# kkbwilldo/quantizations

Hardware: AMD Instinct MI355X
Metric: decode tokens/sec Llama-3-8B NF4 bs=1; 4096×4096 GEMV GB/s vs HBM peak (higher is better)
Workload: dtype f16 activations x 4-bit NF4 weights (exact NF4 codes (fp32 as hi+lo fp16)), fp32 accumulate; 1 GPU; llama3-8b-nf4-dq-decode-bs1; layers=32, prompt_len=32, global_batch=1, stream_batch=1, decode=hipgraph, parallelism=single, projection_groups=64, layer_ops=229, compute_dtype=fp32, rmsnorm_in_grouped_gemv=True, decode_attention=qz_decode_attention, silu_in_gate_up_launch=True, residual_in_gemv_epilogue=True, lm_head=layer_ops.gemv_dense, lm_head_rows_split=False, attention=single GPU

## Files before the change

### quantizations_amd/csrc/diag_stamps.hip

```cpp
#define QZ_STAMPS 1
#include "gemv.hip"

#define QZ_DIAG_API extern "C" __attribute__((visibility("default")))

QZ_DIAG_API int qz_diag_set_stamp_buffer(unsigned long long *buf) {
  return (int)hipMemcpyToSymbol(HIP_SYMBOL(g_qz_stamp), &buf, sizeof(buf));
}

QZ_DIAG_API int qz_diag_gemv_stamped(int M, int K, const void *x, const unsigned char *B, int exact,
                                     const unsigned char *qabsmax, const float *absmax2, const float *code2,
                                     const float *offset, void *y, int *nwaves, void *stream) {
  GemvParams p;
  bool vec_ok;
  const int st = make_params(M, K, x, QZ_DT_F16, B, QZ_NF4, 64, nullptr, qabsmax, absmax2, code2, offset, 256, 0,
                             nullptr, nullptr, y, &p, &vec_ok);
  if (st != QZ_OK) return st;
  if (!vec_ok || !full_steps(K, 64, 256, true, 0) || !nwaves) return QZ_ERR_SHAPE;
  int R, WK;
  choose_geometry(M, K, QZ_DT_F16, &R, &WK);
  if (WK != 1 || (R != 2 && R != 4)) return QZ_ERR_SHAPE;
  set_tables(QZ_NF4, nullptr, exact != 0, QZ_DT_F16, &p);
  const unsigned grid = (unsigned)((M + R * 4 - 1) / (R * 4));
  hipStream_t s = (hipStream_t)stream;
  const bool two = two_steps(K, 1, true);
#define QZ_DG(RR, CL_, TWO_) \
  hipLaunchKernelGGL((k_gemv_4bit<true, QZ_DT_F16, RR, 1, 4, true, CL_, false, TWO_, 2>), dim3(grid), dim3(256), 0, s, p)
#define QZ_DG2(RR, CL_) do { if (two) QZ_DG(RR, CL_, true); else QZ_DG(RR, CL_, false); } while (0)
  if (R == 2) { if (exact) QZ_DG2(2, true); else QZ_DG2(2, false); }
  else { if (exact) QZ_DG2(4, true); else QZ_DG2(4, false); }
#undef QZ_DG2
#undef QZ_DG
  QZ_LAUNCH_CHECK();
  *nwaves = (int)grid * 4;
  return QZ_OK;
}
```

### quantizations_amd/csrc/gemv.hip

```cpp
#include "gemv_launch.h"

namespace qz {

static int env_int(const char *name, int dflt) {
  const char *e = getenv(name);
  return e && *e ? atoi(e) : dflt;
}
static Knobs read_knobs() {
  Knobs k;
  k.wide8 = env_int("QZ_GEMV_WIDE8", 1) != 0;
  const int nr = env_int("QZ_GROUPED_NORM_R", 0);
  k.norm_r = (nr == 1 || nr == 2 || nr == 4) ? nr : 0;
  const int pr = env_int("QZ_PAIR_R", 0);
  k.pair_r = (pr == 2 || pr == 3 || pr == 4 || pr == 6 || pr == 8) ? pr : 0;
  k.pair_wt = env_int("QZ_PAIR_WT", 1) != 0;
  k.pair_ps = env_int("QZ_PAIR_PS", -1);
  k.pair_wk1 = env_int("QZ_PAIR_WK1", 2);
  return k;
}
static Knobs g_knobs = read_knobs();
Knobs &gemv_knobs() { return g_knobs; }
static int g_gemm16_sched = env_int("QZ_GEMM16_SCHED", 971);
int &gemm16_sched() { return g_gemm16_sched; }


template <bool DQ, int DT, int R, bool CL, bool NRM, bool TWO, bool PS = false, bool WT = false>
__global__ __launch_bounds__(256) void k_gemv_4bit_pair(GemvGroup g) {
  const int wave = __builtin_amdgcn_readfirstlane((int)threadIdx.x / kWave);
  const GemvParams seg = g.seg[wave >> 1];
  gemv_body<DQ, DT, R, 1, 4, true, CL, WT, NRM, true, TWO, PS>(seg, blockIdx.x, g.seg);
}

}

using namespace qz;

extern "C" int qz_gemv_4bit(int M, int K, const void *x, int dtype, const unsigned char *B, int quant_type,
                            int blocksize, const float *absmax, const unsigned char *qabsmax, const float *absmax2,
                            const float *code2, const float *offset, int blocksize2, long long block_base,
                            const float *lut, const void *bias, void *y, void *stream) {
  return gemv_impl<false>(M, K, x, dtype, B, quant_type, blocksize, absmax, qabsmax, absmax2, code2, offset,
                          blocksize2, block_base, lut, bias, nullptr, nullptr, y, stream);
}

extern "C" int qz_gemv_4bit_residual(int M, int K, const void *x, int dtype, const unsigned char *B, int quant_type,
                                     int blocksize, const float *absmax, const unsigned char *qabsmax,
                                     const float *absmax2, const float *code2, const float *offset, int blocksize2,
                                     long long block_base, const float *lut, const void *bias, const void *residual,
                                     void *y, void *stream) {
  if (!residual) return QZ_ERR_ARG;
  return gemv_impl<false>(M, K, x, dtype, B, quant_type, blocksize, absmax, qabsmax, absmax2, code2, offset,
                          blocksize2, block_base, lut, bias, residual, nullptr, y, stream);
}

extern "C" int qz_gemv_4bit_grouped(int nseg, const qz_gemv_segment *segs, int K, const void *x, int dtype,
                                    int quant_type, int blocksize, int blocksize2, const float *lut, void *stream) {
  return gemv_grouped_impl<false>(nseg, segs, nullptr, nullptr, K, x, dtype, quant_type, blocksize, blocksize2, lut,
                                  nullptr, 0.0f, stream);
}

extern "C" int qz_gemv_4bit_grouped_rmsnorm(int nseg, const qz_gemv_segment *segs, int K, const void *x, int dtype,
                                            int quant_type, int blocksize, int blocksize2, const float *lut,
                                            const void *norm_weight, float eps, void *stream) {
  if (!norm_weight || !x) return QZ_ERR_ARG;
  return gemv_grouped_impl<false>(nseg, segs, nullptr, nullptr, K, x, dtype, quant_type, blocksize, blocksize2, lut,
                                  norm_weight, eps, stream);
}

template <bool DQ, int DT, int R, bool CL, bool NRM>
static void launch_pair_wt(unsigned grid, size_t lds, hipStream_t s, const GemvGroup &g, bool two) {
  if constexpr (CL && NRM && DT == QZ_DT_F16 && (R == 2 || R == 4)) {
    if (two) hipLaunchKernelGGL((k_gemv_4bit_pair<DQ, DT, R, CL, NRM, true, true, true>), dim3(grid), dim3(256), lds, s, g);
    else hipLaunchKernelGGL((k_gemv_4bit_pair<DQ, DT, R, CL, NRM, false, true, true>), dim3(grid), dim3(256), lds, s, g);
  }
}

template <bool DQ, int DT, int R, bool CL, bool NRM>
static void launch_pair_ps_loop(unsigned grid, int blocks, size_t lds, hipStream_t s, const GemvGroup &g) {
  if constexpr (NRM)
    hipLaunchKernelGGL((k_gemv_4bit_pair<DQ, DT, R, CL, NRM, false, true>), dim3(grid), dim3(256), lds, s, g);
  else
    hipLaunchKernelGGL((k_gemv_4bit_pair<DQ, DT, R, CL, NRM, false>), dim3(blocks), dim3(256), lds, s, g);
}

extern "C" int qz_gemv_4bit_pair_silu(const qz_gemv_segment *segs, int K, const void *x, int dtype, int quant_type,
                                      int blocksize, int blocksize2, const float *lut, const void *norm_weight,
                                      float eps, void *h, void *stream) {
  if (!segs || !h || !x) return QZ_ERR_ARG;
  if (segs[0].M != segs[1].M) return QZ_ERR_SHAPE;
  if (dtype != QZ_DT_F16 && dtype != QZ_DT_BF16) return QZ_ERR_SHAPE;
  GemvGroup g;
  g.nseg = 2;
  const bool cl = exact_codes(quant_type, lut) && dtype == QZ_DT_F16;
  const bool dq = segs[0].qabsmax != nullptr;
  for (int i = 0; i < 2; ++i) {
// ... 1 lines not shown
    bool v;
    const int st = make_params(q.M, K, x, dtype, q.B, quant_type, blocksize, q.absmax, q.qabsmax, q.absmax2, q.code2,
                               q.offset, blocksize2, q.block_base, lut, q.bias, h, &g.seg[i], &v);
    if (st != QZ_OK) return st;
    if ((q.qabsmax != nullptr) != dq || !v || !full_steps(K, blocksize, blocksize2, dq, q.block_base))
      return QZ_ERR_SHAPE;
    set_tables(quant_type & ~QZ_EXACT_CODES, lut, cl, dtype, &g.seg[i]);
    g.seg[i].nw = norm_weight;
    g.seg[i].eps = eps;
  }
  const int M = segs[0].M;
  if (M == 0) return QZ_OK;
  if (norm_weight && (K % 8 != 0 || K > 16384 || ((uintptr_t)x | (uintptr_t)norm_weight) % 16 != 0))
    return QZ_ERR_SHAPE;
  int R, WK;
  choose_geometry(2 * M, K, dtype, &R, &WK);
  if (WK != 1) {
    const int wk1 = gemv_knobs().pair_wk1;
    if (wk1 == 0 || (norm_weight && wk1 != 2)) return QZ_ERR_SHAPE;
    WK = 1;
  }
  if (gemv_knobs().pair_r) R = gemv_knobs().pair_r;
  const int blocks = (M + 2 * R - 1) / (2 * R);
  if (norm_weight && blocks > kNormMaxBlocks) return QZ_ERR_SHAPE;
  for (int i = 2; i < kMaxSeg; ++i) g.start[i] = 0;
  hipStream_t s = (hipStream_t)stream;
  const size_t lds = norm_weight ? (size_t)K * 2 : 0;
  const bool two = two_steps(K, 1, true);
  const int cus = device_cus();
  const size_t img = norm_weight ? (size_t)K * 2 : 0;
  const int per_cu_wt = (int)std::min<size_t>(3, kLdsPerCU / (2 * kTabDwords * 4 + img + 4096));
  const int per_cu = (int)std::min<size_t>(3, kLdsPerCU / (kTabDwords * 4 + img + 4096));
  const bool wt_ok = cl && norm_weight && (R == 2 || R == 4) && blocks >= 3 * 2 * cus && per_cu_wt >= 2 &&
                     gemv_knobs().pair_wt;
  int pgrid_i = 0;
  if (gemv_knobs().pair_ps >= 0) {
    const int ps = gemv_knobs().pair_ps;
    pgrid_i = ps <= 0 ? 0 : ps <= 8 ? cus * ps : ps;
  } else if (norm_weight) {
    pgrid_i = (wt_ok ? 2 : per_cu) * cus;
  }
  const unsigned pgrid = (unsigned)max(pgrid_i, 1);
  const bool persist = pgrid_i > 0 && pgrid_i < blocks;
  const bool pair_wt = persist && wt_ok;
#define QZ_PS(DQ_, DT_, RR, CL_, NRM_)                                                                               \
  do {                                                                                                              \
    if (pair_wt) launch_pair_wt<DQ_, DT_, RR, CL_, NRM_>(pgrid, lds, s, g, two);                                        \
    else if (persist && two) hipLaunchKernelGGL((k_gemv_4bit_pair<DQ_, DT_, RR, CL_, NRM_, true, true>), dim3(pgrid), \
                                                dim3(256), lds, s, g);                                              \
    else if (persist) launch_pair_ps_loop<DQ_, DT_, RR, CL_, NRM_>(pgrid, blocks, lds, s, g);                      \
    else if (two) hipLaunchKernelGGL((k_gemv_4bit_pair<DQ_, DT_, RR, CL_, NRM_, true>), dim3(blocks), dim3(256),    \
                                     lds, s, g);                                                                    \
    else hipLaunchKernelGGL((k_gemv_4bit_pair<DQ_, DT_, RR, CL_, NRM_, false>), dim3(blocks), dim3(256), lds, s, g); \
  } while (0)
#define QZ_PS_R(DQ_, DT_, CL_, NRM_)                  \
  do {                                                \
    if (R == 4) QZ_PS(DQ_, DT_, 4, CL_, NRM_);        \
    else if (R == 8) QZ_PS(DQ_, DT_, 8, CL_, NRM_);   \
    else if (R == 6) QZ_PS(DQ_, DT_, 6, CL_, NRM_);   \
    else if (R == 3) QZ_PS(DQ_, DT_, 3, CL_, NRM_);   \
    else if (R == 1) QZ_PS(DQ_, DT_, 1, CL_, NRM_);   \
    else QZ_PS(DQ_, DT_, 2, CL_, NRM_);               \
  } while (0)
#define QZ_PS_N(DQ_, DT_, CL_)                                                         \
  do {                                                                                 \
    if (norm_weight) QZ_PS_R(DQ_, DT_, CL_, true); else QZ_PS_R(DQ_, DT_, CL_, false); \
  } while (0)
  if (dtype == QZ_DT_F16) {
    if (dq) { if (cl) QZ_PS_N(true, QZ_DT_F16, true); else QZ_PS_N(true, QZ_DT_F16, false); }
    else { if (cl) QZ_PS_N(false, QZ_DT_F16, true); else QZ_PS_N(false, QZ_DT_F16, false); }
  } else {
    if (dq) QZ_PS_N(true, QZ_DT_BF16, false); else QZ_PS_N(false, QZ_DT_BF16, false);
  }
#undef QZ_PS_N
#undef QZ_PS_R
#undef QZ_PS
  QZ_LAUNCH_CHECK();
  return QZ_OK;
}

extern "C" int qz_gemv_knobs(char *buf, int n) {
  char tmp[320];
  const int len = snprintf(tmp, sizeof(tmp),
                           "{\"QZ_GEMV_WIDE8\": %d, \"QZ_GROUPED_NORM_R\": %d, \"QZ_PAIR_R\": %d, \"QZ_PAIR_WT\": %d, "
                           "\"QZ_PAIR_PS\": %d, \"QZ_PAIR_WK1\": %d, \"QZ_GEMM16_SCHED\": %d, \"cus\": %d}",
                           gemv_knobs().wide8, gemv_knobs().norm_r, gemv_knobs().pair_r, gemv_knobs().pair_wt,
                           gemv_knobs().pair_ps, gemv_knobs().pair_wk1, gemm16_sched(), device_cus());
  if (buf && n > len) memcpy(buf, tmp, (size_t)len + 1);
  return len;
}

extern "C" int qz_gemv_set_knob(const char *name, int value) {
  if (!name) return QZ_ERR_ARG;
  Knobs &k = gemv_knobs();
  if (!strcmp(name, "QZ_GEMV_WIDE8")) k.wide8 = value != 0;
  else if (!strcmp(name, "QZ_GROUPED_NORM_R")) k.norm_r = (value == 1 || value == 2 || value == 4) ? value : 0;
  else if (!strcmp(name, "QZ_PAIR_R")) k.pair_r = (value == 2 || value == 3 || value == 4 || value == 6 || value == 8) ? value : 0;
  else if (!strcmp(name, "QZ_PAIR_WT")) k.pair_wt = value != 0;
  else if (!strcmp(name, "QZ_PAIR_PS")) k.pair_ps = value;
  else if (!strcmp(name, "QZ_PAIR_WK1")) k.pair_wk1 = value;
  else if (!strcmp(name, "QZ_GEMM16_SCHED")) gemm16_sched() = value;
  else return QZ_ERR_ARG;
  return QZ_OK;
}
```

### quantizations_amd/csrc/gemv_core.h

```cpp
#pragma once
#include "common.h"

#include <atomic>
#include <cstdio>
#include <cstdlib>
#include <cstring>

namespace qz {

constexpr int kTabCopies = 32;
constexpr int kTabDwords = 256 * kTabCopies;
constexpr int kTabCopiesCL = 16;

constexpr uint16_t f16_bits_rne_c(float f) {
  const uint32_t u = __builtin_bit_cast(uint32_t, f);
  const uint32_t sign = (u >> 16) & 0x8000u, au = u & 0x7FFFFFFFu;
  if (au == 0) return (uint16_t)sign;
  const uint32_t e = (au >> 23) - 127u + 15u, m = au & 0x7FFFFFu;
  uint32_t h = (e << 10) | (m >> 13);
  const uint32_t rem = m & 0x1FFFu;
  if (rem > 0x1000u || (rem == 0x1000u && (h & 1u))) h += 1u;
  return (uint16_t)(sign | h);
}
struct ByteTable {
// ... 324 lines not shown
    store_byte_table_entry<PIECES>(s_tab, u32x4{h, l, h, l}, (uint32_t)e);
  }
}

template <int NT, int PIECES = kTabCopies / 4>
__device__ __forceinline__ void build_byte_table_f32(uint32_t *s_tab, const float *lut) {
  for (int e = threadIdx.x; e < 256; e += NT) {
    const uint32_t a = __float_as_uint(lut[e >> 4]), b = __float_as_uint(lut[e & 15]);
    store_byte_table_entry<PIECES>(s_tab, u32x4{a, b, a, b}, (uint32_t)e);
  }
}

template <bool DQ, int DT, int R, bool NOX, bool FS> struct StepLoads {
  static constexpr int kXWords = DT == QZ_DT_F32 ? 32 : 16;
  u32x4 wv[R];
  uint32_t q[R];
  float a[R];
  uint32_t xr[kXWords];
  int xb;
  bool on;

  __device__ __forceinline__ void load_x(const void *x, uint32_t e0) {
    const u32x4 *p = reinterpret_cast<const u32x4 *>(reinterpret_cast<const char *>(x) +
                                                     e0 * (DT == QZ_DT_F32 ? 4u : 2u));
#pragma unroll
    for (int i = 0; i < kXWords / 4; ++i) {
      const u32x4 v = p[i];
      xr[4 * i] = v.x; xr[4 * i + 1] = v.y; xr[4 * i + 2] = v.z; xr[4 * i + 3] = v.w;
    }
  }

  __device__ __forceinline__ void issue(const GemvParams &p, int row0, int s, int lane, int row_bytes) {
    if constexpr (FS) {
      issue_full(p, row0, s, lane, row_bytes);
      return;
    }
    const uint32_t boff_raw = ((uint32_t)s << 10) + ((uint32_t)lane << 4);
    on = boff_raw < (uint32_t)row_bytes;
    const uint32_t boff = on ? boff_raw : 0u;
    xb = 2 * (int)boff;
    if constexpr (!NOX) load_x(p.x, 2u * boff);
#pragma unroll
    for (int r = 0; r < R; ++r) {
      const uint32_t row = (uint32_t)min(row0 + r, p.M - 1);
      const unsigned char *rowp = p.B + (size_t)row * (uint32_t)row_bytes;
      wv[r] = __builtin_nontemporal_load(reinterpret_cast<const u32x4 *>(rowp + boff));
      const uint32_t b = (uint32_t)p.block_base + ((row * (uint32_t)p.K + 2u * boff) >> p.bs_log2);
      if constexpr (DQ) {
        q[r] = p.sc.qabsmax[b];
        a[r] = p.sc.absmax2[b >> p.bs2_log2];
      } else {
        a[r] = p.sc.absmax[b];
      }
    }
  }

  __device__ __forceinline__ void issue_full(const GemvParams &p, int row0, int s, int lane, int row_bytes) {
    const uint32_t boff = ((uint32_t)s << 10) + ((uint32_t)lane << 4);
    on = true;
    xb = 2 * (int)boff;
    if constexpr (!NOX) load_x(p.x, 2u * boff);
    const uint32_t lb = (2u * boff) >> p.bs_log2;
    const uint32_t sb = ((uint32_t)s << 11) >> p.bs_log2;
    const uint32_t bpr = (uint32_t)p.K >> p.bs_log2;
#pragma unroll
    for (int r = 0; r < R; ++r) {
      const uint32_t row = (uint32_t)min(row0 + r, p.M - 1);
      const unsigned char *rowp = p.B + (size_t)row * (uint32_t)row_bytes;
      wv[r] = __builtin_nontemporal_load(reinterpret_cast<const u32x4 *>(rowp + boff));
      const uint32_t rb = (uint32_t)p.block_base + row * bpr;
      if constexpr (DQ) {
        q[r] = (p.sc.qabsmax + rb)[lb];
        typedef const __attribute__((address_space(4))) float *cfp;
        a[r] = ((cfp)p.sc.absmax2)[(rb + sb) >> p.bs2_log2];
      } else {
        a[r] = (p.sc.absmax + rb)[lb];
      }
    }
  }
};

template <int DT> __device__ __forceinline__ float norm_chunk_ss(const u32x4 &v, float ss) {
  const uint32_t w[4] = {v.x, v.y, v.z, v.w};
#pragma unroll
  for (int j = 0; j < 8; ++j) {
    const uint32_t b = (w[j >> 1] >> (16 * (j & 1))) & 0xFFFFu;
    const float h = DT == QZ_DT_F16 ? __half2float(__ushort_as_half((unsigned short)b)) : __uint_as_float(b << 16);
    ss = __fadd_rn(ss, __fmul_rn(h, h));
  }
  return ss;
}
__device__ __forceinline__ float norm_wave_sum(float v) {
#pragma unroll
  for (int o = 32; o > 0; o >>= 1) v += __shfl_xor(v, o, kWave);
  return v;
}
template <int DT> __device__ __forceinline__ u32x4 norm_chunk_apply(const u32x4 &xv, const u32x4 &wv, float rs) {
  const uint32_t xw[4] = {xv.x, xv.y, xv.z, xv.w}, ww[4] = {wv.x, wv.y, wv.z, wv.w};
  uint32_t o[4];
#pragma unroll
  for (int d = 0; d < 4; ++d) {
    float r2[2];
#pragma unroll
    for (int h = 0; h < 2; ++h) {
      const uint32_t xb = (xw[d] >> (16 * h)) & 0xFFFFu, wb = (ww[d] >> (16 * h)) & 0xFFFFu;
      float xs = __fmul_rn(DT == QZ_DT_F16 ? __half2float(__ushort_as_half((unsigned short)xb)) : __uint_as_float(xb << 16),
                           rs);
      asm volatile("" : "+v"(xs));
      if constexpr (DT == QZ_DT_F16) {
        const float hn = __half2float(__float2half_rn(xs));
        r2[h] = __fmul_rn(__half2float(__ushort_as_half((unsigned short)wb)), hn);
      } else {
        const float hn = __bfloat162float(__float2bfloat16(xs));
        r2[h] = __fmul_rn(__uint_as_float(wb << 16), hn);
      }
      asm volatile("" : "+v"(r2[h]));
    }
    if constexpr (DT == QZ_DT_F16)
      o[d] = (uint32_t)__half_as_ushort(__float2half_rn(r2[0])) | ((uint32_t)__half_as_ushort(__float2half_rn(r2[1])) << 16);
    else
      o[d] = (uint32_t)__bfloat16_as_ushort(__float2bfloat16(r2[0])) |
             ((uint32_t)__bfloat16_as_ushort(__float2bfloat16(r2[1])) << 16);
  }
  return u32x4{o[0], o[1], o[2], o[3]};
}
__device__ __forceinline__ uint32_t norm_x_off(uint32_t chunk) {
  const uint32_t s = chunk >> 8, l = (chunk >> 2) & 63u, i = chunk & 3u;
  return (s << 12) + (l << 6) + ((i ^ ((l >> 2) & 3u)) << 4);
}

constexpr int kMaxSeg = 4;
struct GemvGroup {
  GemvParams seg[kMaxSeg];
  int start[kMaxSeg];
  int nseg;
  int total;
};
struct LoraGroup {
  LoraOp seg[kMaxSeg];
};

template <bool DQ, int DT, int R, int WK, int NW, bool FS, bool CL, bool WT, bool NRM, bool PAIR, bool TWO, bool PS,
          int STAMP = 0, bool LORA = false>
__device__ __forceinline__ void gemv_body(const GemvParams &p_in, const int block, const GemvParams *pair = nullptr,
                                          const LoraOp *lora = nullptr) {
  static_assert(!LORA || (!PAIR && DT != QZ_DT_F32), "adapter operand: single / grouped launches, 16-bit activations");
  static_assert(!NRM || (NW == 4 && FS && DT != QZ_DT_F32), "fused pre-norm: 4 waves, full steps, 16-bit activations");
  static_assert(!PAIR || (NW == 4 && WK == 1 && DT != QZ_DT_F32), "pair: 4 waves, WK = 1, 16-bit activations");
  static_assert(!PS || (PAIR && FS), "persistent form: pair launches, full steps");
  static_assert(!TWO || (FS && WK == 1), "two-step form: full steps, whole rows per wave");
  static_assert(!CL || DT == QZ_DT_F16, "exact codes are the fp16-activation table");
  static_assert(NW * 64 >= 256, "one byte-table entry per thread");
  constexpr int kPieces = WT ? 16 : kTabCopies / 4;
  QZ_STAMP_DECL;
  QZ_STAMP(0);
  const GemvParams p = load_params(p_in);
  constexpr int RG = NW / WK;
  constexpr bool kBF = DT == QZ_DT_BF16;
  constexpr bool kF32 = DT == QZ_DT_F32;
  constexpr bool kWide = CL || kBF || kF32;
  __shared__ float s_code2[PAIR ? 2 : 1][DQ ? 256 : 1];
  __shared__ float s_part[NW][R];
  __shared__ float s_part2[PS ? 2 : 1][NW][R];
  __shared__ __attribute__((aligned(16))) uint32_t s_tab[(WT ? 2 : 1) * kTabDwords];
  extern __shared__ __attribute__((aligned(16))) unsigned char s_x[];

  const int lane = threadIdx.x & (kWave - 1);
  const int wave = __builtin_amdgcn_readfirstlane(threadIdx.x / kWave);
  const int wk = wave % WK;
  const int rg = wave / WK;
  int row0 = PAIR ? (block * 2 + (wave & 1)) * R : (block * RG + rg) * R;
  const int cb = PAIR ? (wave >> 1) : 0;
  const int row_bytes = p.K >> 1;
  const int nsteps = (row_bytes + 1023) >> 10;

  float c2 = 0.0f, c2b = 0.0f, offset = 0.0f;
  if constexpr (DQ) {
    if constexpr (PAIR) {
      c2 = keep_sp(pair[0].sc.code2)[threadIdx.x];
      c2b = keep_sp(pair[1].sc.code2)[threadIdx.x];
    } else if (NW * 64 == 256 || threadIdx.x < 256) {
      c2 = p.sc.code2[threadIdx.x & 255];
    }
    offset = *p.sc.offset;
  }
  u32x4 tab_entry = {0u, 0u, 0u, 0u};
  if (!p.lut && threadIdx.x < 256) {
    const ByteTable *bt = kF32 ? (p.tabsel ? &g_byte_tab_fp4_f32 : &g_byte_tab_nf4_f32)
                          : kBF ? (p.tabsel ? &g_byte_tab_fp4_bf : &g_byte_tab_nf4_bf)
                                : (CL ? &g_byte_tab_nf4x : (p.tabsel ? &g_byte_tab_fp4 : &g_byte_tab_nf4));
    tab_entry = reinterpret_cast<const u32x4 *>(bt->v)[threadIdx.x];
  }
  constexpr int kNChunks = NRM ? 8 : 1;
  constexpr int kNHeld = NRM ? 2 : 1;
  u32x4 nx[kNChunks], nwh[kNHeld];
  const int n_nchunk = p.K >> 3;
  if constexpr (NRM) {
#pragma unroll
    for (int i = 0; i < kNChunks; ++i) {
      const int c = (int)threadIdx.x + 256 * i;
      if (c < n_nchunk) nx[i] = reinterpret_cast<const u32x4 *>(p.x)[c];
    }
#pragma unroll
    for (int i = 0; i < kNHeld; ++i) {
      const int c = (int)threadIdx.x + 256 * i;
      if (c < n_nchunk) nwh[i] = reinterpret_cast<const u32x4 *>(p.nw)[c];
    }
    __builtin_amdgcn_sched_barrier(0);
  }
  typedef StepLoads<DQ, DT, R, NRM, FS> Loads;
  Loads cur, other;
  int s = wk;
  cur.issue(p, row0, s < nsteps ? s : 0, lane, row_bytes);
  float lo_b[LORA ? R : 1], lo_t = 0.0f;
  bool lo_on = false;
  if constexpr (LORA) {
    const int lr = keep_s(lora->r);
    const char *lB = reinterpret_cast<const char *>(keep_sp(lora->B));
    const float *lt = keep_sp(lora->t);
    lo_on = lane < lr && wk == 0;
    const int j = lo_on ? lane : 0;
    lo_t = lt[j];
#pragma unroll
    for (int r = 0; r < R; ++r) {
      const size_t row = (size_t)min(row0 + r, p.M - 1);
      lo_b[r] = load_f32<DT>(lB + row * (size_t)lr * 2u, j);
    }
  }
  const bool have = s < nsteps;
  const int n_my = have ? (nsteps - wk + WK - 1) / WK : 0;
  if constexpr (DQ) {
    if (NW * 64 == 256 || threadIdx.x < 256) s_code2[0][threadIdx.x & 255] = c2;
    if constexpr (PAIR) s_code2[PAIR ? 1 : 0][threadIdx.x] = c2b;
  }
  __shared__ float s_nss[NRM ? 4 : 1];
  if constexpr (NRM) {
    float ss = 0.0f;
#pragma unroll
    for (int i = 0; i < kNChunks; ++i)
      if ((int)threadIdx.x + 256 * i < n_nchunk) ss = norm_chunk_ss<DT>(nx[i], ss);
    ss = norm_wave_sum(ss);
    if (lane == 0) s_nss[wave] = ss;
  }
  float out_scale = p.out_scale;
  if constexpr (kF32) {
    if (p.lut) {
      out_scale = 1.0f;
      build_byte_table_f32<NW * 64, kPieces>(s_tab, p.lut);
    } else if (threadIdx.x < 256) {
      store_byte_table_entry<kPieces>(s_tab, tab_entry);
    }
  } else if constexpr (kBF) {
    if (p.lut) {
      out_scale = 1.0f;
      build_byte_table_bf16<NW * 64, kPieces>(s_tab, p.lut);
    } else if (threadIdx.x < 256) {
      store_byte_table_entry<kPieces>(s_tab, tab_entry);
    }
  } else if constexpr (CL) {
    if (p.lut) {
      const int S = lut_shift(p.lut);
      out_scale = ldexpf(1.0f, -S);
      build_byte_table_exact<NW * 64, kPieces>(s_tab, p.lut, S);
    } else if (threadIdx.x < 256 && (STAMP & 48) == 0) {
      store_byte_table_entry<kPieces>(s_tab, tab_entry);
    }
  } else if (threadIdx.x < 256) {
    store_byte_table_entry<kPieces>(s_tab, tab_entry);
  }
  if constexpr ((STAMP & 32) == 0) __syncthreads();
  if constexpr (NRM) {
    const float tot = __fadd_rn(__fadd_rn(s_nss[0], s_nss[1]), __fadd_rn(s_nss[2], s_nss[3]));
    const float rs = rsqrtf(__fadd_rn(__fmul_rn(tot, 1.0f / (float)p.K), p.eps));
#pragma unroll
    for (int i = 0; i < kNChunks; ++i) {
      const int c = (int)threadIdx.x + 256 * i;
      if (c < n_nchunk) {
        const u32x4 xv = i < kNHeld ? nx[i] : reinterpret_cast<const u32x4 *>(p.x)[c];
        const u32x4 wv = i < kNHeld ? nwh[i < kNHeld ? i : 0] : reinterpret_cast<const u32x4 *>(p.nw)[c];
        *reinterpret_cast<u32x4 *>(s_x + norm_x_off((uint32_t)c)) = norm_chunk_apply<DT>(xv, wv, rs);
      }
    }
    __syncthreads();
  }
  QZ_STAMP(1);
  const uint32_t jb = WT ? (kWide ? (uint32_t)(lane & 31) << 3 : (uint32_t)lane << 2)
                        : (kWide ? (uint32_t)(lane & (kTabCopiesCL - 1)) << 3 : (uint32_t)(lane & 31) << 2);

  float acc[R];
#pragma unroll
  for (int r = 0; r < R; ++r) acc[r] = 0.0f;

  auto consume = [&](const Loads &c) {
    if constexpr (NRM) {
      auto &xr = const_cast<Loads &>(c).xr;
      const uint32_t c0 = (uint32_t)c.xb >> 3;
#pragma unroll
      for (int i = 0; i < 4; ++i) {
        const u32x4 v = *reinterpret_cast<const u32x4 *>(s_x + norm_x_off(c0 + (uint32_t)i));
        xr[4 * i] = v.x; xr[4 * i + 1] = v.y; xr[4 * i + 2] = v.z; xr[4 * i + 3] = v.w;
      }
    }
#pragma unroll
    for (int r = 0; r < R; ++r) {
      float am;
      if constexpr (DQ) am = __fadd_rn(__fmul_rn(s_code2[cb][c.q[r]], c.a[r]), offset);
      else am = c.a[r];
      am = c.on ? am : 0.0f;
      float d;
      if constexpr (kF32) {
        d = chunk_dot_tab_f32(c.wv[r], c.xr, s_tab, jb);
      } else {
        d = chunk_dot_tab<kWide, WT, kBF>(c.wv[r], c.xr, s_tab, jb);
      }
      acc[r] = fmaf(d, am, acc[r]);
    }
  };
  if constexpr (PS) {
    auto pair_out = [&](int blk, int par) {
      float v[R];
#pragma unroll
      for (int r = 0; r < R; ++r) v[r] = wave_sum_last(acc[r]);
      if (lane == kWave - 1) {
#pragma unroll
        for (int r = 0; r < R; ++r) {
          float o = v[r] * out_scale;
          if (p.bias) o += load_f32<DT>(p.bias, min(row0 + r, p.M - 1));
          s_part2[par][wave][r] = o;
        }
      }
      __syncthreads();
      if ((int)threadIdx.x < 2 * R) {
        const int g2 = threadIdx.x / R, r = threadIdx.x % R;
        const int row = (blk * 2 + g2) * R + r;
        if (row < p.M) {
          const float gv = round_store<DT>(s_part2[par][g2][r]), uv = round_store<DT>(s_part2[par][2 + g2][r]);
          const float a = round_store<DT>(__fdiv_rn(gv, __fadd_rn(1.0f, expf(-gv))));
          store_f32<DT>(keep_sp(pair[0].y), row, __fmul_rn(a, uv));
        }
      }
    };
    const int nblocks = (p.M + 2 * R - 1) / (2 * R);
    int blk = block;
    for (int it = 0;; ++it) {
      if constexpr (TWO) {
        other.issue(p, row0, s + WK, lane, row_bytes);
        __builtin_amdgcn_sched_barrier(0);
        consume(cur);
        consume(other);
      } else {
        const int n = n_my;
        other.issue(p, row0, n >= 2 ? 1 : 0, lane, row_bytes);
        __builtin_amdgcn_sched_barrier(0);
        int j = 0, ss = 0;
        for (; j + 3 < n; j += 2) {
          consume(cur);
          cur.issue(p, row0, ss + 2, lane, row_bytes);
          __builtin_amdgcn_sched_barrier(0);
          consume(other);
          other.issue(p, row0, ss + 3, lane, row_bytes);
// ... 101 lines not shown
          if (p.bias) {
            o0 += load_f32<DT>(p.bias, row0 + r);
            o1 += load_f32<DT>(p.bias, row0 + r + 1);
          }
          o0 = add_res<DT>(o0, p.res, row0 + r);
          o1 = add_res<DT>(o1, p.res, row0 + r + 1);
          reinterpret_cast<uint32_t *>(p.y)[(row0 + r) >> 1] = pack16<DT>(o0, o1);
        }
      } else {
#pragma unroll
        for (int r = 0; r < R; ++r) {
          const int row = row0 + r;
          if (row < p.M) {
            float o = v[r] * out_scale;
            if (p.bias) o += load_f32<DT>(p.bias, row);
            o = add_res<DT>(o, p.res, row);
            store_f32<DT>(p.y, row, o);
          }
        }
      }
    }
    QZ_STAMP(4);
    QZ_STAMP_FLUSH(block * NW + wave);
    return;
  }
#pragma unroll
  for (int r = 0; r < R; ++r) {
    const float v = wave_sum_last(acc[r]);
    if (lane == kWave - 1) s_part[wave][r] = v;
  }
  __syncthreads();
  if ((int)threadIdx.x < RG * R) {
    const int g = threadIdx.x / R, r = threadIdx.x % R;
    const int row = (block * RG + g) * R + r;
    if (row < p.M) {
      float v = 0.0f;
#pragma unroll
      for (int k = 0; k < WK; ++k) v += s_part[g * WK + k][r];
      v *= out_scale;
      if (p.bias) v += load_f32<DT>(p.bias, row);
      store_f32<DT>(p.y, row, add_res<DT>(v, p.res, row));
    }
  }
}

template <bool DQ, int DT, bool LORA = false>
__device__ __forceinline__ void gemv_generic_body(const GemvParams &p, int quant_type, const LoraOp *lora = nullptr) {
  __shared__ float s_lut[16];
  if (threadIdx.x < 16) s_lut[threadIdx.x] = p.lut ? p.lut[threadIdx.x] : 0.0f;
  __syncthreads();
  const int lane = threadIdx.x & (kWave - 1);
  const int row = blockIdx.x * 4 + threadIdx.x / kWave;
  if (row >= p.M) return;
  const float offset = DQ ? *p.sc.offset : 0.0f;
  float acc = 0.0f;
  for (int k = lane; k < p.K; k += kWave) {
    const long long e = (long long)row * p.K + k;
    const uint32_t byte = p.B[e >> 1];
    const uint32_t nib = (e & 1) ? (byte & 0xFu) : (byte >> 4);
    const long long b = p.block_base + (e >> p.bs_log2);
    float am;
    if constexpr (DQ) am = __fadd_rn(__fmul_rn(p.sc.code2[p.sc.qabsmax[b]], p.sc.absmax2[b >> p.bs2_log2]), offset);
    else am = p.sc.absmax[b];
    float c;
    if (p.lut) c = s_lut[nib];
    else if (quant_type == QZ_NF4) c = kNF4[nib];
    else c = (nib & 8u ? -1.0f : 1.0f) * dequant_fp4_tree(nib & 7u, 1.0f);
    acc = fmaf(load_f32<DT>(p.x, k), __fmul_rn(c, am), acc);
  }
  if constexpr (LORA) {
    if (lane < lora->r) acc = fmaf(load_f32<DT>(lora->B, (long long)row * lora->r + lane), lora->t[lane], acc);
  }
  acc = wave_sum_last(acc);
  if (lane == kWave - 1) {
    if (p.bias) acc += load_f32<DT>(p.bias, row);
    store_f32<DT>(p.y, row, add_res<DT>(acc, p.res, row));
  }
}


struct Knobs {
  int wide8;
  int norm_r;
  int pair_r;
  int pair_wt;
  int pair_ps;
  int pair_wk1;
};
constexpr int kNormMaxBlocks = 4096;
constexpr long long kNormSplitMaxValues = 1LL << 23;
constexpr size_t kLdsPerCU = 160 * 1024;
Knobs &gemv_knobs();

static int ilog2(long long v) {
  int l = 0;
  while ((1LL << l) < v) ++l;
  return (1LL << l) == v ? l : -1;
}

static inline bool two_steps(int K, int WK, bool fs) { return fs && WK == 1 && K == 2 * 2048; }

static void choose_geometry(int M, int K, int dtype, int *R, int *WK) {
  const int nsteps = ((K >> 1) + 1023) >> 10;
  const bool f32 = dtype == QZ_DT_F32;
  *R = (f32 || (long long)M * K > (1LL << 26)) ? 4 : 2;
  *WK = 1;
  if (*R == 4 && nsteps == 4 && !f32) *WK = 2;
  const long long min_waves = f32 ? 1024 : 2048;
  while ((long long)((M + *R - 1) / *R) * (*WK) < min_waves) {
    if (*R > 1) *R >>= 1;
    else if (*WK < 4 && *WK * 2 <= nsteps) *WK <<= 1;
    else break;
  }
}

static bool full_steps(int K, int blocksize, int blocksize2, bool dq, long long block_base) {
  if (K % 2048 != 0 || K % blocksize != 0) return false;
  const long long step_blocks = blocksize >= 2048 ? 1 : 2048 / blocksize;
  if (block_base % step_blocks != 0) return false;
  return !dq || blocksize2 % step_blocks == 0;
}

static void set_tables(int quant_type, const float *lut, bool cl, int dtype, GemvParams *p) {
  const bool fp4 = !lut && quant_type == QZ_FP4;
  p->tabsel = fp4 ? 1 : (cl && dtype == QZ_DT_F16 ? 2 : 0);
  p->out_scale = fp4 ? 1.0f / 12.0f : 1.0f;
  if (dtype == QZ_DT_F16 && cl && !lut) p->out_scale = 1.0f / (float)(1 << kNF4ExactShift);
}

static bool exact_codes(int quant_type_flags, const float *lut) {
  if (lut) return true;
  return (quant_type_flags & QZ_EXACT_CODES) && (quant_type_flags & ~QZ_EXACT_CODES) == QZ_NF4;
}

static int make_params(int M, int K, const void *x, int dtype, const unsigned char *B, int quant_type, int blocksize,
                       const float *absmax, const unsigned char *qabsmax, const float *absmax2, const float *code2,
                       const float *offset, int blocksize2, long long block_base, const float *lut, const void *bias,
                       void *y, GemvParams *p, bool *vec_ok) {
  if (!x || !B || !y || M < 0 || K < 0) return QZ_ERR_ARG;
  quant_type &= ~QZ_EXACT_CODES;
  if ((absmax == nullptr) == (qabsmax == nullptr)) return QZ_ERR_ARG;
  const bool dq = qabsmax != nullptr;
  if (dq && (!absmax2 || !code2 || !offset)) return QZ_ERR_ARG;
  if (quant_type != QZ_FP4 && quant_type != QZ_NF4) return QZ_ERR_DTYPE;
  if (dtype != QZ_DT_F16 && dtype != QZ_DT_BF16 && dtype != QZ_DT_F32) return QZ_ERR_DTYPE;
  const int bsl = ilog2(blocksize);
  const int bs2l = dq ? ilog2(blocksize2) : 0;
  if (bsl < 1 || bs2l < 0) return QZ_ERR_BLOCKSIZE;
  p->B = B;
  p->x = x;
  p->sc = ScaleSrc{absmax, qabsmax, absmax2, code2, offset, blocksize2};
  p->bias = bias;
  p->y = y;
  p->lut = lut;
  p->block_base = block_base;
  p->M = M;
  p->K = K;
  p->bs_log2 = bsl;
  p->bs2_log2 = bs2l;
  p->out_scale = 1.0f;
  p->tabsel = 0;
  p->nw = nullptr;
  p->eps = 0.0f;
  p->res = nullptr;
  *vec_ok = K > 0 && (K % 32) == 0 && blocksize >= 32 && (reinterpret_cast<uintptr_t>(B) % 16) == 0 &&
            (reinterpret_cast<uintptr_t>(x) % 16) == 0 &&
// ... 7 lines not shown
```

### quantizations_amd/csrc/gemv_launch.h

```cpp
#pragma once
#include "gemv_core.h"

namespace qz {

template <bool DQ, int DT, int R, int WK, int NW, bool FS, bool CL, bool WT, bool TWO, int STAMP = 0>
__global__ __launch_bounds__(NW * 64) void k_gemv_4bit(GemvParams p) {
  gemv_body<DQ, DT, R, WK, NW, FS, CL, WT, false, false, TWO, false, STAMP>(p, blockIdx.x);
}

template <bool DQ, int DT, int R, int WK, int NW, bool FS, bool CL, bool WT, bool TWO>
__global__ __launch_bounds__(NW * 64) void k_gemv_4bit_lora(GemvParams p, LoraOp l) {
  gemv_body<DQ, DT, R, WK, NW, FS, CL, WT, false, false, TWO, false, 0, true>(p, blockIdx.x, nullptr, &l);
}

template <bool DQ, int DT, int R, int WK, bool FS, bool CL, bool NRM, bool TWO>
__global__ __launch_bounds__(256) void k_gemv_4bit_grouped(GemvGroup g) {
  const int b = blockIdx.x;
  int s = 0;
#pragma unroll
  for (int i = 1; i < kMaxSeg; ++i)
    if (i < g.nseg && b >= g.start[i]) s = i;
  s = __builtin_amdgcn_readfirstlane(s);
  const GemvParams seg = g.seg[s];
  const int start = g.start[s];
  gemv_body<DQ, DT, R, WK, 4, FS, CL, false, NRM, false, TWO, false>(seg, b - start);
}

template <bool DQ, int DT, int R, int WK, bool FS, bool CL, bool NRM, bool TWO>
__global__ __launch_bounds__(256) void k_gemv_4bit_grouped_lora(GemvGroup g, LoraGroup lg) {
  const int b = blockIdx.x;
  int s = 0;
#pragma unroll
  for (int i = 1; i < kMaxSeg; ++i)
    if (i < g.nseg && b >= g.start[i]) s = i;
  s = __builtin_amdgcn_readfirstlane(s);
  const GemvParams seg = g.seg[s];
  const LoraOp lo = lg.seg[s];
  const int start = g.start[s];
  gemv_body<DQ, DT, R, WK, 4, FS, CL, false, NRM, false, TWO, false, 0, true>(seg, b - start, nullptr, &lo);
}

template <bool DQ, int DT>
__global__ __launch_bounds__(256) void k_gemv_4bit_generic(GemvParams p, int quant_type) {
  gemv_generic_body<DQ, DT>(p, quant_type);
}

template <bool DQ, int DT>
__global__ __launch_bounds__(256) void k_gemv_4bit_generic_lora(GemvParams p, int quant_type, LoraOp l) {
  gemv_generic_body<DQ, DT, true>(p, quant_type, &l);
}


template <bool LORA, bool DQ, int DT, int R, int WK, int NW, bool FS, bool CL, bool WT, bool TWO>
static void launch_gemv(unsigned grid, hipStream_t s, const GemvParams &p, const LoraOp *l) {
  if constexpr (LORA)
    hipLaunchKernelGGL((k_gemv_4bit_lora<DQ, DT, R, WK, NW, FS, CL, WT, TWO>), dim3(grid), dim3(NW * 64), 0, s, p, *l);
  else hipLaunchKernelGGL((k_gemv_4bit<DQ, DT, R, WK, NW, FS, CL, WT, TWO>), dim3(grid), dim3(NW * 64), 0, s, p);
}

template <bool LORA, bool DQ, int DT, int R, int WK, bool FS, bool CL, bool NRM, bool TWO>
static void launch_grouped(int blocks, size_t lds, hipStream_t s, const GemvGroup &g, const LoraGroup &lg) {
  if constexpr (LORA)
    hipLaunchKernelGGL((k_gemv_4bit_grouped_lora<DQ, DT, R, WK, FS, CL, NRM, TWO>), dim3(blocks), dim3(256), lds, s,
                       g, lg);
  else hipLaunchKernelGGL((k_gemv_4bit_grouped<DQ, DT, R, WK, FS, CL, NRM, TWO>), dim3(blocks), dim3(256), lds, s, g);
}

template <bool LORA, bool DQ>
static int launch_generic(const GemvParams &p, int quant_type, const LoraOp *l, int dtype, hipStream_t s) {
  const unsigned grid = (unsigned)((p.M + 3) / 4);
#define QZ_GG(DT_)                                                                                               \
  do {                                                                                                           \
    if constexpr (LORA)                                                                                          \
      hipLaunchKernelGGL((k_gemv_4bit_generic_lora<DQ, DT_>), dim3(grid), dim3(256), 0, s, p, quant_type, *l);   \
    else hipLaunchKernelGGL((k_gemv_4bit_generic<DQ, DT_>), dim3(grid), dim3(256), 0, s, p, quant_type);         \
  } while (0)
  if (dtype == QZ_DT_F16) QZ_GG(QZ_DT_F16);
  else if (dtype == QZ_DT_BF16) QZ_GG(QZ_DT_BF16);
  else if constexpr (!LORA) QZ_GG(QZ_DT_F32);
  else return QZ_ERR_DTYPE;
#undef QZ_GG
  return QZ_OK;
}

template <bool LORA, bool DQ, int DT, bool FS, bool CL>
static void launch_vec(const GemvParams &p, const LoraOp *l, int R, int WK, hipStream_t s) {
  const int RG = 4 / WK;
  const unsigned grid = (unsigned)((p.M + R * RG - 1) / (R * RG));
#define QZ_GV(RR, WW, TWO_) launch_gemv<LORA, DQ, DT, RR, WW, 4, FS, CL, false, (WW == 1 && TWO_)>(grid, s, p, l)
#define QZ_GV_RW(TWO_)                        \
  do {                                        \
    if (R == 4 && WK == 2) QZ_GV(4, 2, TWO_); \
    else if (R == 4) QZ_GV(4, 1, TWO_);       \
    else if (R == 2) QZ_GV(2, 1, TWO_);       \
    else if (WK == 1) QZ_GV(1, 1, TWO_);      \
    else if (WK == 2) QZ_GV(1, 2, TWO_);      \
    else QZ_GV(1, 4, TWO_);                   \
  } while (0)
  if constexpr (FS) {
    if (two_steps(p.K, WK, true)) { QZ_GV_RW(true); return; }
  }
  if constexpr (FS && CL && DT == QZ_DT_F16) {
    if (WK == 1 && (R == 2 || R == 4) && p.K >= 14336 && gemv_knobs().wide8) {
      const unsigned g8 = (unsigned)((p.M + R * 8 - 1) / (R * 8));
      if (R == 4) launch_gemv<LORA, DQ, DT, 4, 1, 8, FS, CL, true, false>(g8, s, p, l);
      else launch_gemv<LORA, DQ, DT, 2, 1, 8, FS, CL, true, false>(g8, s, p, l);
      return;
    }
// ... 37 lines not shown
  p.res = res;
  if (M == 0) return QZ_OK;
  const bool dq = qabsmax != nullptr;
  hipStream_t s = (hipStream_t)stream;
  const bool cl = exact_codes(quant_type, lut) && dtype == QZ_DT_F16;
  quant_type &= ~QZ_EXACT_CODES;
  int rc;
  if (!vec_ok) {
    if (K == 0) return QZ_ERR_SHAPE;
    rc = dq ? launch_generic<LORA, true>(p, quant_type, l, dtype, s) : launch_generic<LORA, false>(p, quant_type, l, dtype, s);
  } else {
    int R, WK;
    choose_geometry(M, K, dtype, &R, &WK);
    set_tables(quant_type, lut, cl, dtype, &p);
    const bool fs = full_steps(K, blocksize, blocksize2, dq, block_base);
    rc = cl ? dispatch_tab<LORA, true>(p, l, dtype, dq, fs, R, WK, s) : dispatch_tab<LORA, false>(p, l, dtype, dq, fs, R, WK, s);
  }
  if (rc != QZ_OK) return rc;
  QZ_LAUNCH_CHECK();
  return QZ_OK;
}

template <bool LORA>
static int gemv_grouped_impl(int nseg, const qz_gemv_segment *segs, const qz_lora_segment *lora, const float *t,
                             int K, const void *x, int dtype, int quant_type, int blocksize, int blocksize2,
                             const float *lut, const void *nw, float eps, void *stream) {
  if (nseg < 1 || nseg > QZ_GEMV_MAX_SEGMENTS || !segs) return QZ_ERR_ARG;
  GemvGroup g;
  LoraGroup lg;
  g.nseg = nseg;
  const bool cl = exact_codes(quant_type, lut) && dtype == QZ_DT_F16;
  bool all_vec = true;
  long long total_m = 0;
  const bool dq = segs[0].qabsmax != nullptr;
  for (LoraOp &o : lg.seg) o = LoraOp{t, t, 0};
  for (int i = 0; i < nseg; ++i) {
    const qz_gemv_segment &q = segs[i];
    bool v;
    const int st = make_params(q.M, K, x, dtype, q.B, quant_type, blocksize, q.absmax, q.qabsmax, q.absmax2, q.code2,
                               q.offset, blocksize2, q.block_base, lut, q.bias, q.y, &g.seg[i], &v);
    if (st != QZ_OK) return st;
    if ((q.qabsmax != nullptr) != dq) return QZ_ERR_ARG;
    if constexpr (LORA) {
      if (lora[i].B) {
        if (lora[i].r < 1 || lora[i].r > QZ_LORA_MAX_RANK || lora[i].t_offset < 0) return QZ_ERR_ARG;
        lg.seg[i] = LoraOp{lora[i].B, t + lora[i].t_offset, lora[i].r};
      }
    }
    all_vec = all_vec && v;
    total_m += q.M;
  }
  if (total_m == 0) return QZ_OK;
  if (nw) {
    if (!all_vec || total_m > INT32_MAX || (dtype != QZ_DT_F16 && dtype != QZ_DT_BF16) || K % 8 != 0 || K > 16384 ||
        ((uintptr_t)x | (uintptr_t)nw) % 16 != 0)
      return QZ_ERR_SHAPE;
    for (int i = 0; i < nseg; ++i) {
      if (!full_steps(K, blocksize, blocksize2, dq, segs[i].block_base)) return QZ_ERR_SHAPE;
      g.seg[i].nw = nw;
      g.seg[i].eps = eps;
    }
  }
  if (!all_vec || total_m > INT32_MAX) {
    for (int i = 0; i < nseg; ++i) {
      const qz_gemv_segment &q = segs[i];
      if constexpr (LORA) {
        if (lora[i].B) {
          const int rc = qz_gemv_4bit_lora(q.M, K, x, dtype, q.B, quant_type, blocksize, q.absmax, q.qabsmax,
                                           q.absmax2, q.code2, q.offset, blocksize2, q.block_base, lut, q.bias,
                                           nullptr, lora[i].B, lora[i].r, t + lora[i].t_offset, q.y, stream);
          if (rc != QZ_OK) return rc;
          continue;
        }
      }
      const int rc = qz_gemv_4bit(q.M, K, x, dtype, q.B, quant_type, blocksize, q.absmax, q.qabsmax, q.absmax2,
                                  q.code2, q.offset, blocksize2, q.block_base, lut, q.bias, q.y, stream);
      if (rc != QZ_OK) return rc;
    }
    return QZ_OK;
  }
  int R, WK;
  choose_geometry((int)total_m, K, dtype, &R, &WK);
  if (nw && gemv_knobs().norm_r && WK == 1) R = gemv_knobs().norm_r;
  const int rows_per_block = R * (4 / WK);
  int blocks = 0;
  for (int i = 0; i < nseg; ++i) {
    set_tables(quant_type & ~QZ_EXACT_CODES, lut, cl, dtype, &g.seg[i]);
    g.start[i] = blocks;
    blocks += (g.seg[i].M + rows_per_block - 1) / rows_per_block;
  }
  for (int i = nseg; i < kMaxSeg; ++i) g.start[i] = blocks;
  g.total = blocks;
  if (nw && blocks > kNormMaxBlocks) return QZ_ERR_SHAPE;
  if (nw && WK != 1 && (long long)blocks * K > kNormSplitMaxValues) return QZ_ERR_SHAPE;
  bool all_fs = true;
  for (int i = 0; i < nseg; ++i) all_fs = all_fs && full_steps(K, blocksize, blocksize2, dq, segs[i].block_base);
  hipStream_t s = (hipStream_t)stream;
  const bool two = two_steps(K, WK, all_fs || nw);
  const size_t lds = nw ? (size_t)K * 2 : 0;
#define QZ_GR1(DQ_, DT_, RR, WW, FS_, CL_, NRM_)                                                                  \
  do {                                                                                                            \
    if (FS_ && two && WW == 1)                                                                                    \
      launch_grouped<LORA, DQ_, DT_, RR, WW, FS_, CL_, NRM_, (FS_ && WW == 1)>(blocks, lds, s, g, lg);            \
    else launch_grouped<LORA, DQ_, DT_, RR, WW, FS_, CL_, NRM_, false>(blocks, lds, s, g, lg);                    \
  } while (0)
#define QZ_GR_RW(DQ_, DT_, FS_, CL_, NRM_)                         \
  do {                                                             \
    if (R == 4 && WK == 2) QZ_GR1(DQ_, DT_, 4, 2, FS_, CL_, NRM_); \
    else if (R == 4) QZ_GR1(DQ_, DT_, 4, 1, FS_, CL_, NRM_);       \
    else if (R == 2) QZ_GR1(DQ_, DT_, 2, 1, FS_, CL_, NRM_);       \
    else if (WK == 1) QZ_GR1(DQ_, DT_, 1, 1, FS_, CL_, NRM_);      \
    else if (WK == 2) QZ_GR1(DQ_, DT_, 1, 2, FS_, CL_, NRM_);      \
    else QZ_GR1(DQ_, DT_, 1, 4, FS_, CL_, NRM_);                   \
  } while (0)
#define QZ_GR_DT(DQ_, FS_)                                                                                          \
  do {                                                                                                              \
    if (dtype == QZ_DT_F16) { if (cl) QZ_GR_RW(DQ_, QZ_DT_F16, FS_, true, false); else QZ_GR_RW(DQ_, QZ_DT_F16, FS_, false, false); } \
    else if (dtype == QZ_DT_BF16) QZ_GR_RW(DQ_, QZ_DT_BF16, FS_, false, false);                                     \
    else if constexpr (!LORA) QZ_GR_RW(DQ_, QZ_DT_F32, FS_, false, false);                                          \
    else return QZ_ERR_DTYPE;                                                                                       \
  } while (0)
  if (nw) {
    if (dtype == QZ_DT_F16) {
      if (dq) { if (cl) QZ_GR_RW(true, QZ_DT_F16, true, true, true); else QZ_GR_RW(true, QZ_DT_F16, true, false, true); }
      else { if (cl) QZ_GR_RW(false, QZ_DT_F16, true, true, true); else QZ_GR_RW(false, QZ_DT_F16, true, false, true); }
    } else {
      if (dq) QZ_GR_RW(true, QZ_DT_BF16, true, false, true); else QZ_GR_RW(false, QZ_DT_BF16, true, false, true);
    }
  } else if (all_fs) { if (dq) QZ_GR_DT(true, true); else QZ_GR_DT(false, true); }
  else { if (dq) QZ_GR_DT(true, false); else QZ_GR_DT(false, false); }
#undef QZ_GR_DT
#undef QZ_GR_RW
#undef QZ_GR1
  QZ_LAUNCH_CHECK();
  return QZ_OK;
}

}
```

Baseline: 552.8 tokens/s.

## Add 8-wave grouped RMSNorm GEMV kernel and packed-f16 norm math

```diff
diff --git a/quantizations_amd/csrc/diag_stamps.hip b/quantizations_amd/csrc/diag_stamps.hip
--- a/quantizations_amd/csrc/diag_stamps.hip
+++ b/quantizations_amd/csrc/diag_stamps.hip
@@ -34,3 +34,45 @@
   *nwaves = (int)grid * 4;
   return QZ_OK;
 }
+
+template <int R, bool TWO>
+__global__ __launch_bounds__(256) void k_diag_grouped_norm(GemvGroup g) {
+  const GemvParams seg = g.seg[0];
+  gemv_body<true, QZ_DT_F16, R, 1, 4, true, true, false, true, false, TWO, false, 1>(seg, blockIdx.x);
+}
+
+QZ_DIAG_API int qz_diag_grouped_norm_stamped(int M, int K, const void *x, const unsigned char *B,
+                                             const unsigned char *qabsmax, const float *absmax2, const float *code2,
+                                             const float *offset, const void *norm_weight, float eps, void *y,
+                                             int *nwaves, void *stream) {
+  GemvGroup g;
+  bool vec_ok;
+  const int st = make_params(M, K, x, QZ_DT_F16, B, QZ_NF4, 64, nullptr, qabsmax, absmax2, code2, offset, 256, 0,
+                             nullptr, nullptr, y, &g.seg[0], &vec_ok);
+  if (st != QZ_OK) return st;
+  if (!vec_ok || !full_steps(K, 64, 256, true, 0) || !nwaves || !norm_weight || K > 16384 ||
+      ((uintptr_t)x | (uintptr_t)norm_weight) % 16 != 0)
+    return QZ_ERR_SHAPE;
+  int R, WK;
+  choose_geometry(M, K, QZ_DT_F16, &R, &WK);
+  if (WK != 1 || (R != 2 && R != 4)) return QZ_ERR_SHAPE;
+  set_tables(QZ_NF4, nullptr, true, QZ_DT_F16, &g.seg[0]);
+  g.seg[0].nw = norm_weight;
+  g.seg[0].eps = eps;
+  const int blocks = (M + R * 4 - 1) / (R * 4);
+  if (blocks > kNormMaxBlocks) return QZ_ERR_SHAPE;
+  g.nseg = 1;
+  g.start[0] = 0;
+  for (int i = 1; i < kMaxSeg; ++i) g.start[i] = blocks;
+  g.total = blocks;
+  hipStream_t s = (hipStream_t)stream;
+  const size_t lds = (size_t)K * 2;
+  const bool two = two_steps(K, 1, true);
+#define QZ_DN(RR, TWO_) hipLaunchKernelGGL((k_diag_grouped_norm<RR, TWO_>), dim3(blocks), dim3(256), lds, s, g)
+  if (R == 2) { if (two) QZ_DN(2, true); else QZ_DN(2, false); }
+  else { if (two) QZ_DN(4, true); else QZ_DN(4, false); }
+#undef QZ_DN
+  QZ_LAUNCH_CHECK();
+  *nwaves = blocks * 4;
+  return QZ_OK;
+}
diff --git a/quantizations_amd/csrc/gemv.hip b/quantizations_amd/csrc/gemv.hip
--- a/quantizations_amd/csrc/gemv.hip
+++ b/quantizations_amd/csrc/gemv.hip
@@ -11,6 +11,7 @@
   k.wide8 = env_int("QZ_GEMV_WIDE8", 1) != 0;
   const int nr = env_int("QZ_GROUPED_NORM_R", 0);
   k.norm_r = (nr == 1 || nr == 2 || nr == 4) ? nr : 0;
+  k.norm_nw8 = env_int("QZ_GROUPED_NORM_NW8", 0) != 0;
   const int pr = env_int("QZ_PAIR_R", 0);
   k.pair_r = (pr == 2 || pr == 3 || pr == 4 || pr == 6 || pr == 8) ? pr : 0;
   k.pair_wt = env_int("QZ_PAIR_WT", 1) != 0;
@@ -178,9 +179,9 @@
 extern "C" int qz_gemv_knobs(char *buf, int n) {
   char tmp[320];
   const int len = snprintf(tmp, sizeof(tmp),
-                           "{\"QZ_GEMV_WIDE8\": %d, \"QZ_GROUPED_NORM_R\": %d, \"QZ_PAIR_R\": %d, \"QZ_PAIR_WT\": %d, "
-                           "\"QZ_PAIR_PS\": %d, \"QZ_PAIR_WK1\": %d, \"QZ_GEMM16_SCHED\": %d, \"cus\": %d}",
-                           gemv_knobs().wide8, gemv_knobs().norm_r, gemv_knobs().pair_r, gemv_knobs().pair_wt,
+                           "{\"QZ_GEMV_WIDE8\": %d, \"QZ_GROUPED_NORM_R\": %d, \"QZ_GROUPED_NORM_NW8\": %d, \"QZ_PAIR_R\": %d, "
+                           "\"QZ_PAIR_WT\": %d, \"QZ_PAIR_PS\": %d, \"QZ_PAIR_WK1\": %d, \"QZ_GEMM16_SCHED\": %d, \"cus\": %d}",
+                           gemv_knobs().wide8, gemv_knobs().norm_r, gemv_knobs().norm_nw8, gemv_knobs().pair_r, gemv_knobs().pair_wt,
                            gemv_knobs().pair_ps, gemv_knobs().pair_wk1, gemm16_sched(), device_cus());
   if (buf && n > len) memcpy(buf, tmp, (size_t)len + 1);
   return len;
@@ -191,6 +192,7 @@
   Knobs &k = gemv_knobs();
   if (!strcmp(name, "QZ_GEMV_WIDE8")) k.wide8 = value != 0;
   else if (!strcmp(name, "QZ_GROUPED_NORM_R")) k.norm_r = (value == 1 || value == 2 || value == 4) ? value : 0;
+  else if (!strcmp(name, "QZ_GROUPED_NORM_NW8")) k.norm_nw8 = value != 0;
   else if (!strcmp(name, "QZ_PAIR_R")) k.pair_r = (value == 2 || value == 3 || value == 4 || value == 6 || value == 8) ? value : 0;
   else if (!strcmp(name, "QZ_PAIR_WT")) k.pair_wt = value != 0;
   else if (!strcmp(name, "QZ_PAIR_PS")) k.pair_ps = value;
diff --git a/quantizations_amd/csrc/gemv_core.h b/quantizations_amd/csrc/gemv_core.h
--- a/quantizations_amd/csrc/gemv_core.h
+++ b/quantizations_amd/csrc/gemv_core.h
@@ -430,6 +430,15 @@
 
 template <int DT> __device__ __forceinline__ float norm_chunk_ss(const u32x4 &v, float ss) {
   const uint32_t w[4] = {v.x, v.y, v.z, v.w};
+  if constexpr (DT == QZ_DT_F16) {
+#pragma unroll
+    for (int d = 0; d < 4; ++d) {
+      const h2_t h = __builtin_bit_cast(h2_t, w[d]);
+      ss = __builtin_fmaf((float)h.x, (float)h.x, ss);
+      ss = __builtin_fmaf((float)h.y, (float)h.y, ss);
+    }
+    return ss;
+  }
 #pragma unroll
   for (int j = 0; j < 8; ++j) {
     const uint32_t b = (w[j >> 1] >> (16 * (j & 1))) & 0xFFFFu;
@@ -446,6 +455,16 @@
 template <int DT> __device__ __forceinline__ u32x4 norm_chunk_apply(const u32x4 &xv, const u32x4 &wv, float rs) {
   const uint32_t xw[4] = {xv.x, xv.y, xv.z, xv.w}, ww[4] = {wv.x, wv.y, wv.z, wv.w};
   uint32_t o[4];
+  if constexpr (DT == QZ_DT_F16) {
+#pragma unroll
+    for (int d = 0; d < 4; ++d) {
+      const h2_t xh = __builtin_bit_cast(h2_t, xw[d]);
+      const float x0 = __fmul_rn((float)xh.x, rs), x1 = __fmul_rn((float)xh.y, rs);
+      const h2_t hn = __builtin_bit_cast(h2_t, cvt_pk_f16_rne(x0, x1));
+      o[d] = __builtin_bit_cast(uint32_t, __builtin_bit_cast(h2_t, ww[d]) * hn);
+    }
+    return u32x4{o[0], o[1], o[2], o[3]};
+  }
 #pragma unroll
   for (int d = 0; d < 4; ++d) {
     float r2[2];
@@ -493,7 +512,8 @@
 __device__ __forceinline__ void gemv_body(const GemvParams &p_in, const int block, const GemvParams *pair = nullptr,
                                           const LoraOp *lora = nullptr) {
   static_assert(!LORA || (!PAIR && DT != QZ_DT_F32), "adapter operand: single / grouped launches, 16-bit activations");
-  static_assert(!NRM || (NW == 4 && FS && DT != QZ_DT_F32), "fused pre-norm: 4 waves, full steps, 16-bit activations");
+  static_assert(!NRM || ((NW == 4 || (NW == 8 && !PAIR)) && FS && DT != QZ_DT_F32),
+                "fused pre-norm: 4 waves (8: single / grouped launches), full steps, 16-bit activations");
   static_assert(!PAIR || (NW == 4 && WK == 1 && DT != QZ_DT_F32), "pair: 4 waves, WK = 1, 16-bit activations");
   static_assert(!PS || (PAIR && FS), "persistent form: pair launches, full steps");
   static_assert(!TWO || (FS && WK == 1), "two-step form: full steps, whole rows per wave");
@@ -541,18 +561,21 @@
   }
   constexpr int kNChunks = NRM ? 8 : 1;
   constexpr int kNHeld = NRM ? 2 : 1;
+  constexpr int kNHalves = NRM ? NW / 4 : 1;
   u32x4 nx[kNChunks], nwh[kNHeld];
   const int n_nchunk = p.K >> 3;
+  const int nt = kNHalves == 1 ? (int)threadIdx.x : (int)threadIdx.x & 255;
+  const int nh = kNHalves == 1 ? 0 : wave >> 2;
   if constexpr (NRM) {
 #pragma unroll
     for (int i = 0; i < kNChunks; ++i) {
-      const int c = (int)threadIdx.x + 256 * i;
-      if (c < n_nchunk) nx[i] = reinterpret_cast<const u32x4 *>(p.x)[c];
+      const int c = nt + 256 * i;
+      if (c < n_nchunk && (nh == 0 || i % kNHalves == nh)) nx[i] = reinterpret_cast<const u32x4 *>(p.x)[c];
     }
 #pragma unroll
     for (int i = 0; i < kNHeld; ++i) {
-      const int c = (int)threadIdx.x + 256 * i;
-      if (c < n_nchunk) nwh[i] = reinterpret_cast<const u32x4 *>(p.nw)[c];
+      const int c = nt + 256 * i;
+      if (c < n_nchunk && i % kNHalves == nh) nwh[i] = reinterpret_cast<const u32x4 *>(p.nw)[c];
     }
     __builtin_amdgcn_sched_barrier(0);
   }
@@ -583,12 +606,14 @@
   }
   __shared__ float s_nss[NRM ? 4 : 1];
   if constexpr (NRM) {
-    float ss = 0.0f;
-#pragma unroll
-    for (int i = 0; i < kNChunks; ++i)
-      if ((int)threadIdx.x + 256 * i < n_nchunk) ss = norm_chunk_ss<DT>(nx[i], ss);
-    ss = norm_wave_sum(ss);
-    if (lane == 0) s_nss[wave] = ss;
+    if (kNHalves == 1 || nh == 0) {
+      float ss = 0.0f;
+#pragma unroll
+      for (int i = 0; i < kNChunks; ++i)
+        if (nt + 256 * i < n_nchunk) ss = norm_chunk_ss<DT>(nx[i], ss);
+      ss = norm_wave_sum(ss);
+      if (lane == 0) s_nss[wave] = ss;
+    }
   }
   float out_scale = p.out_scale;
   if constexpr (kF32) {
@@ -622,8 +647,8 @@
     const float rs = rsqrtf(__fadd_rn(__fmul_rn(tot, 1.0f / (float)p.K), p.eps));
 #pragma unroll
     for (int i = 0; i < kNChunks; ++i) {
-      const int c = (int)threadIdx.x + 256 * i;
-      if (c < n_nchunk) {
+      const int c = nt + 256 * i;
+      if (c < n_nchunk && i % kNHalves == nh) {
         const u32x4 xv = i < kNHeld ? nx[i] : reinterpret_cast<const u32x4 *>(p.x)[c];
         const u32x4 wv = i < kNHeld ? nwh[i < kNHeld ? i : 0] : reinterpret_cast<const u32x4 *>(p.nw)[c];
         *reinterpret_cast<u32x4 *>(s_x + norm_x_off((uint32_t)c)) = norm_chunk_apply<DT>(xv, wv, rs);
@@ -891,6 +916,7 @@
 struct Knobs {
   int wide8;
   int norm_r;
+  int norm_nw8;
   int pair_r;
   int pair_wt;
   int pair_ps;
diff --git a/quantizations_amd/csrc/gemv_launch.h b/quantizations_amd/csrc/gemv_launch.h
--- a/quantizations_amd/csrc/gemv_launch.h
+++ b/quantizations_amd/csrc/gemv_launch.h
@@ -24,6 +24,19 @@
   const GemvParams seg = g.seg[s];
   const int start = g.start[s];
   gemv_body<DQ, DT, R, WK, 4, FS, CL, false, NRM, false, TWO, false>(seg, b - start);
+}
+
+template <bool DQ, int DT, int R, bool CL, bool TWO>
+__global__ __launch_bounds__(512) void k_gemv_4bit_grouped_norm8(GemvGroup g) {
+  const int b = blockIdx.x;
+  int s = 0;
+#pragma unroll
+  for (int i = 1; i < kMaxSeg; ++i)
+    if (i < g.nseg && b >= g.start[i]) s = i;
+  s = __builtin_amdgcn_readfirstlane(s);
+  const GemvParams seg = g.seg[s];
+  const int start = g.start[s];
+  gemv_body<DQ, DT, R, 1, 8, true, CL, true, true, false, TWO, false>(seg, b - start);
 }
 
 template <bool DQ, int DT, int R, int WK, bool FS, bool CL, bool NRM, bool TWO>
@@ -227,7 +240,16 @@
   int R, WK;
   choose_geometry((int)total_m, K, dtype, &R, &WK);
   if (nw && gemv_knobs().norm_r && WK == 1) R = gemv_knobs().norm_r;
-  const int rows_per_block = R * (4 / WK);
+  int rows_per_block = R * (4 / WK);
+  bool norm8 = false;
+  if constexpr (!LORA) {
+    if (nw && gemv_knobs().norm_nw8 && cl && R == 2 && WK == 1) {
+      long long b8 = 0;
+      for (int i = 0; i < nseg; ++i) b8 += (g.seg[i].M + 2 * 8 - 1) / (2 * 8);
+      norm8 = b8 >= 256;
+      if (norm8) rows_per_block = 2 * 8;
+    }
+  }
   int blocks = 0;
   for (int i = 0; i < nseg; ++i) {
     set_tables(quant_type & ~QZ_EXACT_CODES, lut, cl, dtype, &g.seg[i]);
@@ -265,7 +287,15 @@
     else if constexpr (!LORA) QZ_GR_RW(DQ_, QZ_DT_F32, FS_, false, false);                                          \
     else return QZ_ERR_DTYPE;                                                                                       \
   } while (0)
-  if (nw) {
+  if (norm8) {
+    if constexpr (!LORA) {
+#define QZ_GN8(DQ_, TWO_) \
+  hipLaunchKernelGGL((k_gemv_4bit_grouped_norm8<DQ_, QZ_DT_F16, 2, true, TWO_>), dim3(blocks), dim3(512), lds, s, g)
+      if (dq) { if (two) QZ_GN8(true, true); else QZ_GN8(true, false); }
+      else { if (two) QZ_GN8(false, true); else QZ_GN8(false, false); }
+#undef QZ_GN8
+    }
+  } else if (nw) {
     if (dtype == QZ_DT_F16) {
       if (dq) { if (cl) QZ_GR_RW(true, QZ_DT_F16, true, true, true); else QZ_GR_RW(true, QZ_DT_F16, true, false, true); }
       else { if (cl) QZ_GR_RW(false, QZ_DT_F16, true, true, true); else QZ_GR_RW(false, QZ_DT_F16, true, false, true); }
```

Result: faster. 558.8 tokens/s (median of 6 runs) (+1.1%).
